# yknishidate/single-file-vulkan-pathtracing

Hardware: AMD Instinct MI355X
Metric: Mrays/s, Cornell Box 1920x1080 @ 8 bounces (ms/frame in ms_per_step) (higher is better)
Workload: dtype f32; 1 GPU; C2: CornellBox-Original.obj 1920x1080, 32 spp/frame x 774 frames, 8 bounces, fused pipeline (library default); pipeline=fused

## Files before the change

single-file-vulkan-pathtracing_amd/csrc/film_work.hip:

```cpp
#include "wavefront_host.h"

#include <algorithm>
#include <cmath>
#include <string>
#include <vector>

namespace {
using ptw::SPILL_POOL_ENTRIES;

constexpr size_t SLOT_BYTES_QUEUES = 2 * (8 + 16 + 16 + 8) + 16 + 4, SLOT_BYTES_META = 4 + 4;
constexpr size_t SLOT_BYTES = SLOT_BYTES_QUEUES + SLOT_BYTES_META;

struct WorkNeed { size_t slots, color, terms, terms_over, total; };
WorkNeed work_need(uint64_t n_slots, uint32_t groups, uint32_t term_cap, uint32_t term_pcap, bool queues = true, uint32_t tail = 0)
{
    WorkNeed n{};
    const size_t heads = (size_t)std::max<uint64_t>(n_slots, 1);
    n.slots = tail ? heads * tail : heads;
    n.color = groups == 1 ? heads : 0;
    const bool logs = groups > 1 || tail;
    n.terms = logs ? n.slots * (size_t)term_pcap : 0;
    n.terms_over = logs ? n.slots * (size_t)(term_cap - term_pcap) : 0;
    n.total = n.slots * (queues ? SLOT_BYTES : SLOT_BYTES_META) + sizeof(float4) * (n.color + n.terms + n.terms_over) +
              (logs ? sizeof(float4) * (size_t)SPILL_POOL_ENTRIES : 0);
// ... 50 lines not shown
            for (uint32_t tx = 0; tx < tiles_x; tx++)
                if ((tx + ty) % world == rank) tiles.push_back(tx | (ty << 16));
        if (order == 1u) {
            auto ring = [&](uint32_t t) {
                const float cx = 0.5f * (float)tiles_x, cy = 0.5f * (float)tiles_y;
                const float dx = std::fabs(((float)(t & 0xFFFFu) + 0.5f) - cx) / cx, dy = std::fabs(((float)(t >> 16) + 0.5f) - cy) / cy;
                return std::max(dx, dy);
            };
            std::stable_sort(tiles.begin(), tiles.end(), [&](uint32_t a, uint32_t b) { return ring(a) < ring(b); });
        }
        w.tile_order = order;
        w.rank = rank; w.world = world;
        w.n_tiles = (uint32_t)tiles.size();
        w.tile_rect[0] = w.tile_rect[1] = 0; w.tile_rect[2] = w.tile_rect[3] = -1;
        if (order == 1u) w.h_tiles = tiles; else w.h_tiles.clear();
        PT_HIP(ctx, hipMalloc((void **)&w.d_tiles, sizeof(uint32_t) * std::max<size_t>(tiles.size(), 1)));
        if (!tiles.empty())
            PT_HIP(ctx, hipMemcpy(w.d_tiles, tiles.data(), sizeof(uint32_t) * tiles.size(), hipMemcpyHostToDevice));
    }
    const uint64_t n_slots64 = (uint64_t)lanes * groups * w.n_tiles * 64ull;
    if (n_slots64 >= (1ull << 31)) {
        ctx->err = "too many path slots (frames_in_flight x sample_groups x pixels >= 2^31)";
        return PT_ERR_INVALID_ARG;
    }
    if (!w.d_count) PT_HIP(ctx, hipMalloc((void **)&w.d_count, sizeof(uint32_t) * PTW_COUNT_WORDS));
    if (tail && (n_slots64 * tail >= (1ull << 31) || queues || groups != 1)) {
        ctx->err = "head + tail slots: too many tail slots, or not the fused pipeline's one-group shape";
        return PT_ERR_INVALID_ARG;
    }
    const WorkNeed need = work_need(n_slots64, groups, term_cap, term_pcap, queues, tail);
    const size_t ns = need.slots;
    const size_t limit = ctx->mem_budget;
    pt_status rc = PT_OK;
// ... 148 lines not shown
    std::vector<uint32_t> out;
    out.reserve(w.h_tiles.size());
    if (none) {
        out = w.h_tiles;
    } else {
        auto touches = [&](uint32_t t) {
            const int32_t x = (int32_t)(t & 0xFFFFu) * 8, y = (int32_t)(t >> 16) * 8;
            return x <= rect[2] && x + 7 >= rect[0] && y <= rect[3] && y + 7 >= rect[1];
        };
        for (uint32_t t : w.h_tiles) if (touches(t)) out.push_back(t);
        for (uint32_t t : w.h_tiles) if (!touches(t)) out.push_back(t);
    }
    PT_HIP(ctx, hipStreamSynchronize(st));
    PT_HIP(ctx, hipMemcpy(w.d_tiles, out.data(), sizeof(uint32_t) * out.size(), hipMemcpyHostToDevice));
    std::copy(rect, rect + 4, w.tile_rect);
    return PT_OK;
}

pt_status ptw_shape_and_work(pt_film *f, const pt_params *p_in, RenderShape &sh, int launch_class, bool queues)
{
    pt_status rc = PT_OK;
    pt_params p_local = *p_in;
    if (p_local.pipeline == PT_PIPELINE_WAVEFRONT_NEE) p_local.sample_groups = 1;
    const pt_params *p = &p_local;
    for (int attempt = 0; attempt < 12; attempt++) {
        sh = ptw_choose_shape(f, p, launch_class, attempt);
        rc = ptw_ensure_work(f, p->rank, p->world, sh.lanes, sh.groups, sh.term_cap, sh.term_pcap, queues);
        if (rc != PT_ERR_OOM) return rc;
        const bool can_shrink = (p->frames_in_flight == 0 && sh.lanes > 1) || (p->sample_groups == 0 && sh.groups > 1);
        if (!can_shrink) return rc;
// ... 71 lines not shown
```

single-file-vulkan-pathtracing_amd/csrc/fused.hip:

```cpp
#include "wavefront_host.h"

#include <algorithm>

#define PT_EXTEND_TEMPLATES_ONLY
#include "extend_kernel.h"
#include "extend_inst16.h"

#ifdef PT_FUSED_TIMELINE
__device__ unsigned long long *g_fused_timeline = nullptr;
extern "C" int pt_debug_fused_timeline(void *device_u64x4_per_wave)
{
    return (int)hipMemcpyToSymbol(HIP_SYMBOL(g_fused_timeline), &device_u64x4_per_wave, sizeof(void *));
}
#endif

#ifdef PT_FUSED_HIST
__device__ uint32_t *g_fused_hist = nullptr;
extern "C" int pt_debug_fused_hist(void *device_u32_2x8192x16)
{
    return (int)hipMemcpyToSymbol(HIP_SYMBOL(g_fused_hist), &device_u32_2x8192x16, sizeof(void *));
}
#endif

#include "fused_cull.h"
// ... 83 lines not shown
{
    pt_ctx *ctx = s->ctx;
    if (s->n_inst && nee) {
        ctx->err = "PT_PIPELINE_FUSED with PT_FLAG_NEE is for single-level scenes (instanced scenes: PT_PIPELINE_WAVEFRONT_NEE)";
        return PT_ERR_UNSUPPORTED;
    }
    if (s->n_inst) return plan_fused_inst(s, pl, tmin, fp);
    const size_t tables = sizeof(float4) * 5 * (size_t)s->n_tris;
    if (pl.variant != PT_EXTEND_LDS || pl.spill || !(tmin > 0.f) || tables > 16 * 1024) {
        ctx->err = "PT_PIPELINE_FUSED is for single-level scenes whose BVH4, triangles and shading tables fit LDS (the compact "
                   "kernels' class: <= 2047 triangles in <= 24 KB, stack bound <= 16, tmin > 0)";
        return PT_ERR_UNSUPPORTED;
    }
    fp.lds_stack = pl.lds_stack + 1;
    fp.smem = (size_t)fp.lds_stack * FTB * sizeof(uint32_t) + lds_scene_bytes(s->n_wide, s->n_tris) + tables +
              sizeof(uint32_t) * FS_FIELDS * FTB + sizeof(uint32_t) * (FTB / 64) * PT_FUSED_WTILES;
    fp.pairs = pl.pairs;
    fp.block = FTB;
    int per_cu = 0;
    pt_status rcp;
    if (nee) {
        fp.nee = true;
        fp.smem += sizeof(uint32_t) * FS_NEE_FIELDS * FTB;
        rcp = fused_blocks_per_cu(ctx, 2, fp.smem, pl.pairs, per_cu,
                                  [&](int *n) { return ptw_prepare_kernel(ctx, reinterpret_cast<const void *>(pick_fused_nee(pl.pairs)), FTB, fp.smem, n); });
    } else {
        rcp = fused_blocks_per_cu(ctx, 0, fp.smem, pl.pairs, per_cu, [&](int *n) {
            pt_status rc = PT_OK;
            for (int mode = 2; mode >= 0 && rc == PT_OK; mode--) {
                rc = ptw_prepare_kernel(ctx, reinterpret_cast<const void *>(pick_fused(mode, pl.pairs, true)), FTB, fp.smem + FUSED_COUNT_LDS);
                if (rc == PT_OK) rc = ptw_prepare_kernel(ctx, reinterpret_cast<const void *>(pick_fused(mode, pl.pairs, false)), FTB, fp.smem, mode == 0 ? n : nullptr);
// ... 38 lines not shown
```

single-file-vulkan-pathtracing_amd/csrc/fused_kernel.h:

```cpp
#pragma once

#ifndef PT_FUSED_WAVES
#define PT_FUSED_WAVES 6
#endif

#ifndef PT_FUSED_TB
#define PT_FUSED_TB 512
#endif
constexpr int FTB = PT_FUSED_TB;

#ifndef PT_FUSED_BATCH
#define PT_FUSED_BATCH 256
#endif
#ifndef PT_FUSED_BATCH1
#define PT_FUSED_BATCH1 64
#endif
#define PT_FUSED_WTILES (PT_FUSED_BATCH / 64)
#define PT_FUSED_PARTS 8
#define PT_FUSED_PART_STRIDE 32

enum : int { FS_SLOT = 0, FS_CTR, FS_SEED, FS_WR, FS_WG, FS_WB, FS_PXY, FS_A, FS_B, FS_C, FS_MB, FS_FIELDS };
enum : int { FS_NEE_POS = 0, FS_NEE_R, FS_NEE_G, FS_NEE_B, FS_NEE_FIELDS };
#ifndef PT_FUSED_WAVES_NEE
#define PT_FUSED_WAVES_NEE 4
#endif

#ifndef PT_FUSED_NODE_EXIT
#define PT_FUSED_NODE_EXIT 3
#endif
#ifndef PT_FUSED_NODE_EXIT_B
#define PT_FUSED_NODE_EXIT_B 1
#endif
enum FusedBlock : int {
    FB_ITER = 0,
    FB_SHADE,
    FB_HIT,
    FB_MISS,
// ... 55 lines not shown
    float4 *s_shade = s_tri + 9 * (size_t)n_tris;
    float4 *s_frame = s_shade + 3 * (size_t)n_tris;
    lds_u32 *my_state = (lds_u32 *)reinterpret_cast<uint32_t *>(s_frame + 2 * (size_t)n_tris) + threadIdx.x;
    lds_stage_nodes<FTB, true>(s_wide, g_wide, n_wide);
    lds_stage_tris<FTB, true>(s_tri, g_tri4, n_tris, s_shade, g_shade4);
    for (uint32_t i = threadIdx.x; i < 2 * n_tris; i += FTB) s_frame[i] = g_frame4[i];
    __syncthreads();
    const float4 *wide = s_wide, *tri4 = s_tri;
    const float4 *verts = s_tri + 6 * (size_t)n_tris;

    lds_u32 *my_stack32 = (lds_u32 *)reinterpret_cast<uint32_t *>(smem) + FTB + threadIdx.x;
    const int lane = threadIdx.x & 63;

    FusedDev dev;
    dev.kernel_begin();
    lds_u32 *s_fb = (lds_u32 *)reinterpret_cast<uint32_t *>(s_frame + 2 * (size_t)n_tris) + FS_FIELDS * FTB + (FTB / 64) * PT_FUSED_WTILES + (threadIdx.x >> 6) * (2 * FB_N);
    if constexpr (COUNT) {
        if (lane < 2 * FB_N) s_fb[lane] = 0u;
    }
#define PT_FB(B)                                                                                        \
    if constexpr (COUNT) {                                                                              \
        const unsigned long long m_fb = __ballot(1);                                                    \
        if (lane == __ffsll((long long)m_fb) - 1) { s_fb[2 * (B)] += 1u; s_fb[2 * (B) + 1] += (uint32_t)__popcll(m_fb); } \
    }
    bool out_of_slots = false;
    uint32_t n_rays_wave = 0;
    uint32_t n_cull_wave = 0;
    uint32_t w_next = 0, w_end = 0, w_base = 0;
    uint32_t w_part = blockIdx.x % (uint32_t)PT_FUSED_PARTS, w_tried = 0;
    bool w_tails = false;
    const uint32_t n_tail_slots = HYB ? rc.lanes_active * rc.tail * rc.slots_per_lane : 0u;
    const uint32_t part_len = ((n_slots + PT_FUSED_PARTS - 1) / PT_FUSED_PARTS + 63u) & ~63u;
    lds_u32 *s_wtile = (lds_u32 *)reinterpret_cast<uint32_t *>(s_frame + 2 * (size_t)n_tris) + FS_FIELDS * FTB + (threadIdx.x >> 6) * PT_FUSED_WTILES;
    lds_u32 *my_nee = (lds_u32 *)reinterpret_cast<uint32_t *>(s_frame + 2 * (size_t)n_tris) + FS_FIELDS * FTB + (FTB / 64) * PT_FUSED_WTILES + threadIdx.x;
    ptm::f3 inv{}, invf{}, on{}, of{}, orgp{};
    ptm::RayPre pre{};
    uint32_t ax = 0, ay = 0, az = 0, tri_base = 0;
    float best_t = tmax, best_V = 0.f, best_W = 0.f, best_det = 1.f;
    uint32_t best_pos = PT_MISS;
    uint32_t cur = DONE;
    int sp = -1;

    constexpr uint32_t PENDING = 0xFFFFFFFFu;
    auto pop_pending = [&](uint32_t r) -> uint32_t {
        while (__ballot(r == PENDING)) {
            if (r == PENDING) {
                PT_FB(FB_POP)
                sp--;
                const uint32_t e = my_stack32[sp * FTB];
// ... 150 lines not shown
                        w_part = (w_part + 1u) % (uint32_t)PT_FUSED_PARTS;
                        if (++w_tried >= (uint32_t)PT_FUSED_PARTS) {
                            if (HYB && !w_tails && n_tail_slots) {
                                w_tails = true;
                                w_tried = 0;
                                w_part = blockIdx.x % (uint32_t)PT_FUSED_PARTS;
                                continue;
                            }
                            out_of_slots = true;
                            w_end = w_next;
                            break;
                        }
                    }
                    if (out_of_slots) dev.out_of_slots();
                    if (!out_of_slots && (uint32_t)lane < (w_end - w_base + 63u) / 64u) {
                        if (GROUPED || (HYB && w_tails)) {
                            const uint32_t c = slot_base + w_base + 64u * (uint32_t)lane;
                            s_wtile[lane] = tiles[(c - rc.div_spl.div(c) * rc.slots_per_lane) >> 6];
                        } else {
                            s_wtile[lane] = tiles[div_frames.div(((w_base >> 6) + (uint32_t)lane) * (uint32_t)PT_FUSED_PARTS + w_part)];
                        }
                    }
                    __builtin_amdgcn_wave_barrier();
                }
                const uint32_t take = min((uint32_t)__popcll(m_want), w_end - w_next);
                const uint32_t rank = (uint32_t)__popcll(m_want & ((1ull << lane) - 1ull));
                uint32_t cull_n = 0u;
                if (in_blk && sp < 0 && rank < take) {
                    PT_FB(FB_TAKE)
                    const uint32_t mine = w_next + rank;
                    uint32_t f, g, local;
                    if (HYB && w_tails) {
                        const uint32_t lane_slot = rc.div_spl.div(mine);
                        f = rc.div_tail.div(lane_slot); g = lane_slot - f * rc.tail;
                        local = mine - lane_slot * rc.slots_per_lane;
                        slot = rc.n_head + mine;
                    } else if (GROUPED) {
                        slot = slot_base + mine;
                        const uint32_t lane_slot = rc.div_spl.div(slot);
                        f = rc.div_groups.div(lane_slot); g = lane_slot - f * rc.groups;
                        local = slot - lane_slot * rc.slots_per_lane;
                    } else {
                        const uint32_t q = (mine >> 6) * (uint32_t)PT_FUSED_PARTS + w_part;
                        const uint32_t t = div_frames.div(q);
                        f = q - t * rc.lanes_active; g = 0u;
                        local = t * 64u + (mine & 63u);
                        slot = slot_base + f * rc.slots_per_lane + local;
                    }
                    const uint32_t tw = s_wtile[(mine - w_base) >> 6];
                    const uint32_t px = (tw & 0xFFFFu) * 8u + (local & 7u), py = (tw >> 16) * 8u + ((local >> 3) & 7u);
                    const uint32_t sample0 = (HYB && w_tails) ? rc.head_samples + g : g * rc.group_size;
                    const bool in_image = px < rc.width && py < rc.height && f < rc.lanes_active && sample0 < rc.spp;
                    if (in_image && ptc::pixel_culled(rc, px, py)) {
                        PT_FB(FB_CULLED)
                        if (GROUPED) cull_n = ptc::finish_group(rc, rad, slot, g);
                        else if (!(HYB && w_tails)) cull_n = ptc::finish_plain(rc, rad, slot);
                    } else if (in_image) {
                        pxy = px | (py << 16);
                        ctr = sample0;
                        my_state[FS_A * FTB] = 0u;
                        if (!GROUPED) { my_state[FS_B * FTB] = 0u; my_state[FS_C * FTB] = 0u; }
                        my_state[FS_MB * FTB] = (uint32_t)((int32_t)rc.spp * (rc.frame_base + (int32_t)f)) + 1u;
                        sp = 0;
                        need_primary = true;
                        dev.slot_begin();
                    } else if (GROUPED) {
                        rad.nterm[slot] = 0u;
                    } else if (HYB && w_tails) {
                        rad.nterm[slot - rc.n_head] = 0u;
                    }
                }
                w_next += take;
                if (rc.cull_on) {
                    const uint32_t n_c = ptc::rays_finished<GROUPED>(rc, cull_n);
                    n_rays_wave += n_c;
                    n_cull_wave += n_c;
                }
// ... 54 lines not shown
                    if (shadow) {
                        my_nee[FS_NEE_R * FTB] = __float_as_uint(nc.x); my_nee[FS_NEE_G * FTB] = __float_as_uint(nc.y); my_nee[FS_NEE_B * FTB] = __float_as_uint(nc.z);
                    }
                }
                pre = ptm::ray_setup<true>(org, dir);
                inv = { ptm::safe_inv(dir.x), ptm::safe_inv(dir.y), ptm::safe_inv(dir.z) };
                slab_setup(org, inv, invf, on, of);
                ax = inv.x < 0.f ? 48u : 0u;
                ay = inv.y < 0.f ? 48u : 0u;
                az = inv.z < 0.f ? 48u : 0u;
                tri_base = (uint32_t)pre.kz * 3u * n_tris;
                orgp = { ptm::sel3(pre.kz, org.y, org.z, org.x), ptm::sel3(pre.kz, org.z, org.x, org.y), ptm::sel3(pre.kz, org.x, org.y, org.z) };
                best_t = (NEE && shadow) ? nc.w : tmax;
                best_V = 0.f; best_W = 0.f; best_det = 1.f;
                best_pos = PT_MISS;
                cur = 0u;
                sp = 0;
            }
            const uint32_t n_started = (uint32_t)__popcll(__ballot(got_ray));
            n_rays_wave += n_started;
            dev.rays_started(n_started, HYB && w_tails, lane);
        }
        const bool tracing = cur != DONE;
        const unsigned long long m_tracing = __ballot(tracing);
        if (m_tracing == 0ull && __ballot(sp >= 0) == 0ull && out_of_slots) break;

        const int n_have = __popcll(m_tracing);
        if (tracing) { PT_FB(FB_TRACE) }
        {
            bool dn = cur < LEAF_BIT;
            if (__ballot(dn) != 0ull) {
// ... 102 lines not shown
```

single-file-vulkan-pathtracing_amd/csrc/pt_internal.h:

```cpp
#pragma once
#include <hip/hip_runtime.h>
#include <stdint.h>

#include <string>
#include <vector>

#include "../../include/pt_api.h"

constexpr int PT_N_STATS = 24;
constexpr int PT_N_BLOCKS = 32;
constexpr int PT_N_STATS_ALL = PT_N_STATS + 2 * PT_N_BLOCKS;
constexpr int PT_MAX_PIPES = 4;
namespace {
constexpr int TB = 256;
constexpr uint32_t SENTINEL = 0xFFFFFFFFu;
}

struct pt_ctx {
    int device = 0;
    hipStream_t stream = nullptr;
    bool own_stream = false;
    int num_cus = 256;
    std::string err;
    unsigned long long *d_stats = nullptr;
// ... 65 lines not shown
    std::vector<uint32_t> h_light_prim;
    std::vector<float> h_xforms;
    float4 *d_lights_inst = nullptr;
    uint32_t n_lights_inst = 0;
    float light_area_inst = 0.f;
    uint32_t n_inst = 0, n_tlas_wide = 0, tlas_height = 0;
    double tlas_area_lbvh = 0.0, tlas_area_ploc = 0.0;
    float4 *d_inst6 = nullptr;
    float4 *d_inst_frame = nullptr;
    float4 *d_tlas_wide = nullptr;
    uint32_t *d_tlas_prim_of = nullptr;
    uint4 *d_tlas16 = nullptr;
    uint32_t n_tlas16 = 0, tlas16_levels = 0;
    float tlas_norm_c[3]{}, tlas_norm_s[3]{1.f, 1.f, 1.f}, tlas_norm_rs[3]{1.f, 1.f, 1.f};
    float tlas_bmin[3]{}, tlas_bmax[3]{};
};

struct pt_film {
    pt_ctx *ctx = nullptr;
    uint32_t w = 0, h = 0;
    float *d_rgb = nullptr;
    bool own_rgb = true;
    uint8_t *d_bgra = nullptr;
    struct Work {
        uint32_t rank = 0, world = 0, lanes = 0;
        uint32_t tile_order = 0;
        uint32_t groups = 0, term_cap = 0;
        uint32_t tail = 0;
        uint32_t n_tiles = 0;
        uint32_t n_slots = 0;
        uint32_t *d_tiles = nullptr;
        std::vector<uint32_t> h_tiles;
        int32_t tile_rect[4] = { 0, 0, -1, -1 };
        float4 *d_color = nullptr;
        float4 *d_terms = nullptr;
        float4 *d_terms_over = nullptr;
        uint32_t *d_nterm = nullptr;
        uint32_t *d_spill_head = nullptr;
        float4 *d_spill = nullptr;
        uint2 *d_qid[2] = { nullptr, nullptr };
        float4 *d_qstate[2] = { nullptr, nullptr };
        float4 *d_qrayA[2] = { nullptr, nullptr };
        float2 *d_qrayB[2] = { nullptr, nullptr };
        float4 *d_hit = nullptr;
        uint32_t *d_hit_inst = nullptr;
        uint32_t *d_count = nullptr;
// ... 71 lines not shown
```

single-file-vulkan-pathtracing_amd/csrc/render.hip:

```cpp
#include "wavefront_host.h"

#include <cstring>
#include <algorithm>
#include <string>
#include <vector>

namespace {
using namespace ptw;

pt_status check_params(pt_scene *s, pt_film *f, const pt_params *p)
{
    pt_ctx *ctx = s->ctx;
    if (p->width != f->w || p->height != f->h) { ctx->err = "params width/height differ from the film's"; return PT_ERR_INVALID_ARG; }
    if (p->world == 0 || p->rank >= p->world) { ctx->err = "rank/world invalid"; return PT_ERR_INVALID_ARG; }
    if (p->spp_per_frame == 0 || p->spp_per_frame > 0xFFFFu || p->max_depth == 0 || p->max_depth > 0xFFFFu) {
        ctx->err = "spp_per_frame and max_depth must be in 1..65535";
        return PT_ERR_INVALID_ARG;
    }
    if (p->frame < 0 || p->frame_count == 0) { ctx->err = "frame must be >= 0 and frame_count >= 1"; return PT_ERR_INVALID_ARG; }
    if (p->pipeline > PT_PIPELINE_AUTO) { ctx->err = "unknown pipeline"; return PT_ERR_UNSUPPORTED; }
    if (p->pipeline == PT_PIPELINE_FUSED && (p->flags & PT_FLAG_ASYNC)) {
        ctx->err = "the fused pipeline has no asynchronous form";
        return PT_ERR_UNSUPPORTED;
    }
// ... 88 lines not shown
    }
    const float size[2] = { (float)p->width, (float)p->height };
    int32_t r[4];
    for (int k = 0; k < 2; k++) {
        const float a = (lo[k] + 1.0f) * 0.5f * size[k] - 1.0f, b = (hi[k] + 1.0f) * 0.5f * size[k] + 1.0f;
        if (!(a == a) || !(b == b) || b < 0.f || a > size[k]) return;
        r[k] = (int32_t)std::max(a, 0.f);
        r[k + 2] = (int32_t)std::min(b, size[k] - 1.0f);
    }
    std::copy(r, r + 4, rect);
}

void apply_cull(const pt_ctx *ctx, const pt_params *p, const int32_t rect[4], RenderConst &rc)
{
    rc.cull_on = 0u;
    if (rect[2] < rect[0] || rect[3] < rect[1] || ctx->tune.cull == 0 || ((p->flags & PT_FLAG_COUNT_VISITS) && ctx->tune.cull != 1)) return;
    if (!std::isfinite(p->env[0]) || !std::isfinite(p->env[1]) || !std::isfinite(p->env[2])) return;
    rc.cull_on = 1u;
    std::copy(rect, rect + 4, rc.cull);
    for (int k = 0; k < 3; k++) {
        volatile float c = 0.0f;
        for (uint32_t i = 0; i < p->spp_per_frame; i++) c = c + 1.0f * p->env[k];
        rc.cull_sum[k] = c;
    }
}

pt_status job_setup(Job &j)
{
    pt_scene *s = j.s; pt_film *f = j.f; const pt_params *p = j.p; pt_ctx *ctx = j.ctx;
    pt_film::Work &w = f->work;
    const uint32_t lanes = j.sh.lanes, groups = j.sh.groups;
// ... 451 lines not shown
    if (ctx->tune.term_spill >= 0) spill_cap = std::min<uint32_t>(spill_cap, (uint32_t)ctx->tune.term_spill);
    static_assert(sizeof(Radiance) <= sizeof(pt_ctx::h_rad), "pt_ctx::h_rad holds a Radiance");
    Radiance rad{};
    auto set_rad = [&]() -> pt_status {
        rad = { w.d_color, w.d_terms, w.d_terms_over, w.d_nterm, w.d_spill, w.d_spill_head, d_spill_count, spill_cap, d_overflow, static_cast<const Radiance *>(ctx->d_rad) };
        if (std::memcmp(ctx->h_rad, &rad, sizeof(rad)) != 0) {
            std::memcpy(ctx->h_rad, &rad, sizeof(rad));
            PT_HIP(ctx, hipMemcpyAsync(ctx->d_rad, ctx->h_rad, sizeof(rad), hipMemcpyHostToDevice, st));
        }
        return PT_OK;
    };
    rc_ = set_rad();
    if (rc_ != PT_OK) return rc_;
    RenderConst rc = ptw_render_const(p, w, sh);
    apply_cull(ctx, p, rect, rc);
    const bool profile = !nested && (p->flags & PT_FLAG_PROFILE) != 0;
    ctx->stats.extend_variant = pl.variant;
    ctx->stats.pipelines = 1;
    if (!nested) PT_HIP(ctx, hipEventRecord(ctx->ev_a, st));
    std::vector<hipEvent_t> evs;
    size_t ev_used = 0;
    for (uint32_t done = 0; w.n_slots > 0 && done < p->frame_count; done += sh.lanes) {
        rc.frame_base = p->frame + (int32_t)done;
        rc.lanes_active = std::min(sh.lanes, p->frame_count - done);
        unsigned long long *const d_rays_before = ctx->d_stats + 18;
        if (sh.bounded) {
            PT_HIP(ctx, hipMemcpyAsync(d_rays_before, ctx->d_stats, sizeof(unsigned long long), hipMemcpyDeviceToDevice, st));
            PT_HIP(ctx, hipMemcpyAsync(ctx->d_stats + 20, ctx->d_stats + 19, sizeof(unsigned long long), hipMemcpyDeviceToDevice, st));
            PT_HIP(ctx, hipMemsetAsync(d_spill_count, 0, sizeof(unsigned long long), st));
        }
// ... 112 lines not shown
    if (rc_ != PT_OK) return rc_;
    rc_ = check_params(s, f, p_in);
    if (rc_ != PT_OK) return rc_;
    ExtendPlan pl;
    rc_ = ptw_plan_extend(s, p_in->extend, pl);
    if (rc_ != PT_OK) return rc_;
    pt_params p_res = *p_in;
    p_res.pipeline = resolve_pipeline(s, p_in, pl);
    const pt_params *p = &p_res;
    s->ctx->stats.pipeline = p->pipeline;
    if (p->pipeline == PT_PIPELINE_FUSED) return render_fused(s, f, p, pl, false, false);
    return render_wavefront(s, f, p, pl, false);
}

void ptw_subject_rect(const pt_scene *s, const pt_params *p, int32_t rect[4]) { subject_rect(s, p, rect); }

pt_status ptw_trace(pt_scene *s, const float *rays6, uint32_t n, float tmin, float tmax, uint32_t extend, pt_hit *hits)
{
    pt_ctx *ctx = s->ctx;
    hipStream_t st = ctx->stream;
    if (n == 0) return PT_OK;
    ExtendPlan pl;
    pt_status rc_ = ptw_plan_extend(s, extend, pl);
    if (rc_ != PT_OK) return rc_;
    std::vector<float4> a(n);
    std::vector<float2> b(n);
    for (uint32_t i = 0; i < n; i++) {
        const float *r = rays6 + 6 * (size_t)i;
        a[i] = make_float4(r[0], r[1], r[2], r[3]);
        b[i] = make_float2(r[4], r[5]);
// ... 37 lines not shown
```

single-file-vulkan-pathtracing_amd/csrc/scene_build.hip:

```cpp
#include "bvh_build.h"

#include <hip/hip_fp16.h>

#include <algorithm>
#include <cmath>
#include <cstdlib>
#include <cstring>
#include <string>
#include <vector>

namespace {

__global__ __launch_bounds__(TB) void k_gather(const float *__restrict__ vertices, const uint32_t *__restrict__ indices,
                                               uint32_t n_tris, float4 *__restrict__ tri_orig,
                                               float4 *__restrict__ tlo, float4 *__restrict__ thi)
{
    const uint32_t t = blockIdx.x * TB + threadIdx.x;
    float mn[3] = { INFINITY, INFINITY, INFINITY }, mx[3] = { -INFINITY, -INFINITY, -INFINITY };
    if (t < n_tris) {
        float v[3][3];
        for (int c = 0; c < 3; c++) {
            const uint32_t vi = indices[3 * (size_t)t + c];
            for (int k = 0; k < 3; k++) v[c][k] = vertices[3 * (size_t)vi + k];
        }
// ... 71 lines not shown
        for (int k = 0; k < 4; k++) {
            hl[k] = __half_as_ushort(__float2half_rd((l[k] - c[ax]) * rs[ax] - 3.814697265625e-06f));
            hh[k] = __half_as_ushort(__float2half_ru((h[k] - c[ax]) * rs[ax] + 3.814697265625e-06f));
        }
        d[2 * ax + 0] = hl[0] | (hl[1] << 16); d[2 * ax + 1] = hl[2] | (hl[3] << 16);
        d[6 + 2 * ax + 0] = hh[0] | (hh[1] << 16); d[6 + 2 * ax + 1] = hh[2] | (hh[3] << 16);
    }
    const float4 cw = nd[6];
    uint4 *o = out + 4 * (size_t)i;
    o[0] = make_uint4(d[0], d[1], d[2], d[3]);
    o[1] = make_uint4(d[4], d[5], d[6], d[7]);
    o[2] = make_uint4(d[8], d[9], d[10], d[11]);
    o[3] = make_uint4(__float_as_uint(cw.x), __float_as_uint(cw.y), __float_as_uint(cw.z), __float_as_uint(cw.w));
}

static pt_status make_wide16(pt_scene *s)
{
    pt_ctx *ctx = s->ctx;
    hipStream_t st = ctx->stream;
    ptb_norm_box(s->bmin, s->bmax, s->norm_c, s->norm_s, s->norm_rs);
    (void)hipFree(s->d_wide16);
    s->d_wide16 = nullptr;
    PT_HIP(ctx, hipMalloc((void **)&s->d_wide16, 64 * (size_t)s->n_wide));
    k_wide_half<<<(s->n_wide + TB - 1) / TB, TB, 0, st>>>(s->d_wide, s->n_wide, s->norm_c[0], s->norm_c[1], s->norm_c[2], s->norm_rs[0],
                                                         s->norm_rs[1], s->norm_rs[2], reinterpret_cast<uint4 *>(s->d_wide16));
    PT_HIP(ctx, hipStreamSynchronize(st));
    PT_HIP(ctx, hipGetLastError());
    return PT_OK;
}

__global__ __launch_bounds__(TB) void k_tri_boxes(const float4 *__restrict__ tri_orig, uint32_t n, float4 *__restrict__ tlo,
                                                  float4 *__restrict__ thi)
{
    const uint32_t t = blockIdx.x * TB + threadIdx.x;
    if (t >= n) return;
    const float4 a = tri_orig[3 * (size_t)t + 0], b = tri_orig[3 * (size_t)t + 1], c = tri_orig[3 * (size_t)t + 2];
    tlo[t] = make_float4(fminf(fminf(a.x, b.x), c.x), fminf(fminf(a.y, b.y), c.y), fminf(fminf(a.z, b.z), c.z), 0.f);
    thi[t] = make_float4(fmaxf(fmaxf(a.x, b.x), c.x), fmaxf(fmaxf(a.y, b.y), c.y), fmaxf(fmaxf(a.z, b.z), c.z), 0.f);
}

static void free_tree_products(pt_scene *s)
{
    (void)hipFree(s->d_nodes); (void)hipFree(s->d_keys); (void)hipFree(s->d_prim_of); (void)hipFree(s->d_prim_of_sah);
// ... 499 lines not shown
    if (rc == PT_OK && s->d_wide_sah)
        rc = ptb_refit_wide(ctx, 0, s->d_wide_sah, s->n_wide_sah, d_tlo, d_thi, s->d_prim_of_sah, n, pad, s->norm_c, s->norm_rs);
    if (rc == PT_OK && s->d_wide16t)
        rc = ptb_refit_wide(ctx, 1, s->d_wide16t, s->n_wide16t, d_tlo, d_thi, kept, n, pad, s->norm_c, s->norm_rs);
    if (rc == PT_OK && s->d_wide8)
        rc = ptb_refit_wide(ctx, 2, s->d_wide8, s->n_wide8, d_tlo, d_thi, s->d_prim_of8, n, pad, s->norm_c, s->norm_rs);
    if (rc != PT_OK) return rc;
    const uint32_t *order = s->bvh4_builder != 0u ? s->d_prim_of_sah : s->d_prim_of;
    if (s->d_wide8)
        k_pack<<<gt, TB, 0, st>>>(s->d_tri_orig, s->d_faces, s->d_prim_of8, n, s->d_tri4_8, s->d_shade4, s->d_shade64_8, s->d_ke4_8);
    k_pack<<<gt, TB, 0, st>>>(s->d_tri_orig, s->d_faces, order, n, s->d_tri4, s->d_shade4, s->d_shade64, s->d_ke4, s->d_frame4);
    k_wide_half<<<(s->n_wide + TB - 1) / TB, TB, 0, st>>>(s->d_wide, s->n_wide, s->norm_c[0], s->norm_c[1], s->norm_c[2], s->norm_rs[0],
                                                         s->norm_rs[1], s->norm_rs[2], reinterpret_cast<uint4 *>(s->d_wide16));
    PT_HIP(ctx, hipGetLastError());
    PT_HIP(ctx, hipStreamSynchronize(st));
    return PT_OK;
}

static void keep_host_boxes(pt_scene *s, const std::vector<float4> &lo, const std::vector<float4> &hi)
{
    const uint32_t n = s->n_tris;
    s->h_tlo.resize(3 * (size_t)n);
    s->h_thi.resize(3 * (size_t)n);
    for (uint32_t i = 0; i < n; i++) {
        s->h_tlo[3 * i + 0] = lo[i].x; s->h_tlo[3 * i + 1] = lo[i].y; s->h_tlo[3 * i + 2] = lo[i].z;
        s->h_thi[3 * i + 0] = hi[i].x; s->h_thi[3 * i + 1] = hi[i].y; s->h_thi[3 * i + 2] = hi[i].z;
    }
}

static pt_status update_tree_products(pt_scene *s, const float4 *d_tlo, const float4 *d_thi, bool refit)
{
// ... 83 lines not shown
```

single-file-vulkan-pathtracing_amd/csrc/wavefront_host.h:

```cpp
#pragma once
#include "wavefront_types.h"

#include <hip/hip_ext.h>

#include <algorithm>

inline pt_status ptw_reserve_spill(pt_ctx *ctx, size_t bytes)
{
    if (bytes <= ctx->spill_bytes) return PT_OK;
    (void)hipFree(ctx->d_spill);
    ctx->d_spill = nullptr;
    ctx->spill_bytes = 0;
    PT_HIP(ctx, hipMalloc((void **)&ctx->d_spill, bytes));
    ctx->spill_bytes = bytes;
    return PT_OK;
}
inline pt_status ptw_prepare_kernel(pt_ctx *ctx, const void *fn, int block, size_t smem, int *per_cu = nullptr)
{
    if (smem > 48 * 1024) PT_HIP(ctx, hipFuncSetAttribute(fn, hipFuncAttributeMaxDynamicSharedMemorySize, (int)smem));
    if (!per_cu) return PT_OK;
    PT_HIP(ctx, hipOccupancyMaxActiveBlocksPerMultiprocessor(per_cu, fn, block, smem));
    *per_cu = std::max(1, std::min(*per_cu, 8));
    return PT_OK;
}
// ... 70 lines not shown
pt_status ptw_plan_fused(pt_scene *s, const ExtendPlan &pl, float tmin, FusedPlan &fp, bool nee = false);
void ptw_launch_fused(const FusedPlan &fp, bool grouped, const ptw::RenderConst &rc, const uint32_t *tiles, const ptw::Radiance &rad,
                      const pt_scene *s, uint32_t n_slots, uint32_t *next_slot, unsigned long long *stats, float tmin, float tmax,
                      hipStream_t st, hipEvent_t ev0, hipEvent_t ev1);

struct RenderShape {
    uint32_t lanes = 1, groups = 1, group_size = 1, term_cap = 0, term_pcap = 0;
    bool bounded = false;
    uint32_t tail = 0;
};
RenderShape ptw_choose_shape(const pt_film *f, const pt_params *p, int launch_class, int shrink = 0);
pt_status ptw_ensure_work(pt_film *f, uint32_t rank, uint32_t world, uint32_t lanes, uint32_t groups, uint32_t term_cap, uint32_t term_pcap,
                          bool queues = true, uint32_t tail = 0);
pt_status ptw_shape_and_work(pt_film *f, const pt_params *p, RenderShape &sh, int launch_class, bool queues = true);
pt_status ptw_tiles_subject_first(pt_film *f, const int32_t rect[4], hipStream_t st);
uint64_t ptw_workspace_bytes(const pt_film *f);
ptw::RenderConst ptw_render_const(const pt_params *p, const pt_film::Work &w, const RenderShape &sh);
uint64_t ptw_valid_local_pixels(const pt_film *f, const pt_params *p);
void ptw_subject_rect(const pt_scene *s, const pt_params *p, int32_t rect[4]);

const void *ptw_extend_hbm_fn(bool count, bool rec64);
void ptw_launch_extend_hbm(bool count, bool rec64, int grid, size_t smem, hipStream_t st, hipEvent_t ev0, hipEvent_t ev1,
                           const float4 *wide, const uint2 *wide16, const float *norm_c, const float *norm_s,
                           const float *norm_rs, const float4 *tri4, const float4 *rec64_tab, uint32_t n_wide, uint32_t n_tris,
                           const float4 *rayA, const float2 *rayB, float4 *hit, const uint32_t *count_in, uint32_t *count_zero,
                           unsigned long long *stats, uint2 *spill, uint32_t spill_stride, int refill, float tmin,
                           float tmax, int lds_stack, int raw_hit, const uint32_t *perm, const float *ray_tmax);
const void *ptw_extend8_fn(bool count, bool spills, bool waves7);
void ptw_launch_extend8(bool count, bool spills, bool waves7, int grid, size_t smem, hipStream_t st, hipEvent_t ev0, hipEvent_t ev1, const uint4 *nodes8,
                        const float *norm_c, const float *norm_s, const float *norm_rs, const float4 *tri4, const float4 *rec64, const float4 *rayA,
// ... 7 lines not shown
```

Before: 58600 Mrays/s.

## Start primary-ray traversal at a precomputed per-tile BVH leaf

After each BVH build, the host reads back the wide BVH and records which leaf holds each triangle. Per frame, it projects all triangles onto the screen and tags each 8x8 tile that only one leaf covers. The tags are stored in a second plane of the tile buffer and staged through LDS. Primary rays in a tagged tile start traversal at that leaf instead of the root, skipping the top-level walk. This adds host readback and classification work on scene or camera changes, plus extra LDS per block. It relies on a simplified camera projection that must match the device camera model.

```diff
diff --git a/single-file-vulkan-pathtracing_amd/csrc/film_work.hip b/single-file-vulkan-pathtracing_amd/csrc/film_work.hip
--- a/single-file-vulkan-pathtracing_amd/csrc/film_work.hip
+++ b/single-file-vulkan-pathtracing_amd/csrc/film_work.hip
@@ -1,7 +1,9 @@
 #include "wavefront_host.h"
+#include "first_leaf.h"
 
 #include <algorithm>
 #include <cmath>
+#include <cstring>
 #include <string>
 #include <vector>
 
@@ -88,9 +90,12 @@
         w.n_tiles = (uint32_t)tiles.size();
         w.tile_rect[0] = w.tile_rect[1] = 0; w.tile_rect[2] = w.tile_rect[3] = -1;
         if (order == 1u) w.h_tiles = tiles; else w.h_tiles.clear();
-        PT_HIP(ctx, hipMalloc((void **)&w.d_tiles, sizeof(uint32_t) * std::max<size_t>(tiles.size(), 1)));
+        PT_HIP(ctx, hipMalloc((void **)&w.d_tiles, sizeof(uint32_t) * 2 * std::max<size_t>(tiles.size(), 1)));
+        PT_HIP(ctx, hipMemset(w.d_tiles, 0, sizeof(uint32_t) * 2 * std::max<size_t>(tiles.size(), 1)));
         if (!tiles.empty())
             PT_HIP(ctx, hipMemcpy(w.d_tiles, tiles.data(), sizeof(uint32_t) * tiles.size(), hipMemcpyHostToDevice));
+        w.h_order = tiles;
+        w.leaf_gen = 0; w.leaf_stale = false; w.leaf_tiles = 0;
     }
     const uint64_t n_slots64 = (uint64_t)lanes * groups * w.n_tiles * 64ull;
     if (n_slots64 >= (1ull << 31)) {
@@ -269,6 +274,37 @@
     PT_HIP(ctx, hipStreamSynchronize(st));
     PT_HIP(ctx, hipMemcpy(w.d_tiles, out.data(), sizeof(uint32_t) * out.size(), hipMemcpyHostToDevice));
     std::copy(rect, rect + 4, w.tile_rect);
+    w.h_order = out;
+    w.leaf_stale = w.leaf_gen != 0;
+    return PT_OK;
+}
+
+pt_status ptw_tiles_first_leaf(pt_film *f, const pt_scene *s, const pt_params *p, bool on, hipStream_t st)
+{
+    pt_film::Work &w = f->work;
+    pt_ctx *ctx = f->ctx;
+    if (!w.d_tiles || !w.n_tiles) return PT_OK;
+    uint32_t *plane = w.d_tiles + w.n_tiles;
+    on = on && s->h_leaf_of.size() == s->n_tris && w.h_order.size() == w.n_tiles;
+    if (!on) {
+        if (w.leaf_gen != 0 || w.leaf_stale) {
+            PT_HIP(ctx, hipStreamSynchronize(st));
+            PT_HIP(ctx, hipMemset(plane, 0, sizeof(uint32_t) * w.n_tiles));
+        }
+        w.leaf_gen = 0; w.leaf_stale = false; w.leaf_tiles = 0;
+        return PT_OK;
+    }
+    const float cam[6] = { p->cam_origin[0], p->cam_origin[1], p->cam_origin[2], p->cam_target[0], p->cam_target[1], p->cam_target[2] };
+    if (!w.leaf_stale && w.leaf_gen == s->tree_gen && std::memcmp(cam, w.leaf_cam, sizeof(cam)) == 0 && w.leaf_size[0] == p->width && w.leaf_size[1] == p->height)
+        return PT_OK;
+    std::vector<uint32_t> codes(w.n_tiles);
+    w.leaf_tiles = ptf::classify_tiles(s->h_leaf_tri9.data(), s->h_leaf_of.data(), s->n_tris, p->cam_origin, p->cam_target, p->width, p->height,
+                                       w.h_order.data(), w.n_tiles, codes.data());
+    PT_HIP(ctx, hipStreamSynchronize(st));
+    PT_HIP(ctx, hipMemcpy(plane, codes.data(), sizeof(uint32_t) * w.n_tiles, hipMemcpyHostToDevice));
+    w.leaf_gen = s->tree_gen; w.leaf_stale = false;
+    std::memcpy(w.leaf_cam, cam, sizeof(cam));
+    w.leaf_size[0] = p->width; w.leaf_size[1] = p->height;
     return PT_OK;
 }
 
diff --git a/single-file-vulkan-pathtracing_amd/csrc/first_leaf.h b/single-file-vulkan-pathtracing_amd/csrc/first_leaf.h
--- /dev/null
+++ b/single-file-vulkan-pathtracing_amd/csrc/first_leaf.h
@@ -0,0 +1,77 @@
+#pragma once
+#include <stdint.h>
+
+#include <algorithm>
+#include <cmath>
+#include <vector>
+
+namespace ptf {
+
+constexpr uint32_t NONE = 0u;
+
+inline uint32_t classify_tiles(const float *tri9, const uint32_t *leaf_of, uint32_t n_tris, const float cam_origin[3], const float cam_target[3],
+                               uint32_t width, uint32_t height, const uint32_t *tiles, uint32_t n_tiles, uint32_t *codes)
+{
+    std::fill(codes, codes + n_tiles, NONE);
+    const double o[3] = { cam_origin[0], cam_origin[1], cam_origin[2] }, t[3] = { cam_target[0], cam_target[1], cam_target[2] };
+    const double den = t[2] - o[2], size[2] = { (double)width, (double)height };
+    if (!(std::fabs(den) > 0.0) || !n_tris || !width || !height) return 0u;
+    std::vector<double> img(6 * (size_t)n_tris);
+    for (uint32_t i = 0; i < 3 * n_tris; i++) {
+        const float *P = tri9 + 3 * (size_t)i;
+        const double a = ((double)P[2] - o[2]) / den;
+        if (!(a > 1.0e-4)) return 0u;
+        for (int k = 0; k < 2; k++) {
+            const double d = o[k] + ((double)P[k] - o[k]) / a - t[k];
+            const double s = (d + 1.0) * 0.5 * size[k];
+            if (!std::isfinite(s)) return 0u;
+            img[2 * (size_t)i + k] = s;
+        }
+    }
+    const int32_t tiles_x = (int32_t)((width + 7) / 8), tiles_y = (int32_t)((height + 7) / 8);
+    constexpr uint32_t MANY = 0xFFFFFFFFu;
+    std::vector<uint32_t> grid((size_t)tiles_x * tiles_y, NONE);
+    for (uint32_t i = 0; i < n_tris; i++) {
+        const double *v = &img[6 * (size_t)i];
+        double big = 0.0;
+        for (int k = 0; k < 6; k++) big = std::max(big, std::fabs(v[k]));
+        const double slack = 1.0 + big * (1.0 / 1048576.0);
+        const double ylo = std::min({ v[1], v[3], v[5] }), yhi = std::max({ v[1], v[3], v[5] });
+        const int32_t ty0 = (int32_t)std::clamp(std::floor((ylo - slack - 8.0) / 8.0), 0.0, (double)tiles_y),
+                      ty1 = (int32_t)std::clamp(std::ceil((yhi + slack) / 8.0), -1.0, (double)tiles_y - 1.0);
+        for (int32_t ty = ty0; ty <= ty1; ty++) {
+            const double ya = 8.0 * ty - slack, yb = 8.0 * ty + 8.0 + slack;
+            if (yhi < ya || ylo > yb) continue;
+            double xlo = 1.0e300, xhi = -1.0e300;
+            for (int e = 0; e < 3; e++) {
+                const double ax = v[2 * e], ay = v[2 * e + 1], bx = v[2 * ((e + 1) % 3)], by = v[2 * ((e + 1) % 3) + 1];
+                if (ay >= ya && ay <= yb) { xlo = std::min(xlo, ax); xhi = std::max(xhi, ax); }
+                for (const double yl : { ya, yb }) {
+                    if ((ay < yl) != (by < yl)) {
+                        const double x = ax + (bx - ax) * ((yl - ay) / (by - ay));
+                        xlo = std::min(xlo, std::clamp(x, std::min(ax, bx), std::max(ax, bx)));
+                        xhi = std::max(xhi, std::clamp(x, std::min(ax, bx), std::max(ax, bx)));
+                    }
+                }
+            }
+            if (xlo > xhi) continue;
+            const int32_t tx0 = (int32_t)std::clamp(std::floor((xlo - slack - 8.0) / 8.0), 0.0, (double)tiles_x),
+                          tx1 = (int32_t)std::clamp(std::ceil((xhi + slack) / 8.0), -1.0, (double)tiles_x - 1.0);
+            for (int32_t tx = tx0; tx <= tx1; tx++) {
+                if (xhi < 8.0 * tx - slack || xlo > 8.0 * tx + 8.0 + slack) continue;
+                uint32_t &g = grid[(size_t)ty * tiles_x + tx];
+                g = (g == NONE || g == leaf_of[i]) ? leaf_of[i] : MANY;
+            }
+        }
+    }
+    uint32_t n = 0;
+    for (uint32_t k = 0; k < n_tiles; k++) {
+        const uint32_t tx = tiles[k] & 0xFFFFu, ty = tiles[k] >> 16;
+        if ((int32_t)tx >= tiles_x || (int32_t)ty >= tiles_y) continue;
+        const uint32_t g = grid[(size_t)ty * tiles_x + tx];
+        if (g != NONE && g != MANY) { codes[k] = g; n++; }
+    }
+    return n;
+}
+
+}
diff --git a/single-file-vulkan-pathtracing_amd/csrc/fused.hip b/single-file-vulkan-pathtracing_amd/csrc/fused.hip
--- a/single-file-vulkan-pathtracing_amd/csrc/fused.hip
+++ b/single-file-vulkan-pathtracing_amd/csrc/fused.hip
@@ -121,7 +121,7 @@
     }
     fp.lds_stack = pl.lds_stack + 1;
     fp.smem = (size_t)fp.lds_stack * FTB * sizeof(uint32_t) + lds_scene_bytes(s->n_wide, s->n_tris) + tables +
-              sizeof(uint32_t) * FS_FIELDS * FTB + sizeof(uint32_t) * (FTB / 64) * PT_FUSED_WTILES;
+              sizeof(uint32_t) * FS_TAIL_AT;
     fp.pairs = pl.pairs;
     fp.block = FTB;
     int per_cu = 0;
diff --git a/single-file-vulkan-pathtracing_amd/csrc/fused_kernel.h b/single-file-vulkan-pathtracing_amd/csrc/fused_kernel.h
--- a/single-file-vulkan-pathtracing_amd/csrc/fused_kernel.h
+++ b/single-file-vulkan-pathtracing_amd/csrc/fused_kernel.h
@@ -16,11 +16,14 @@
 #define PT_FUSED_BATCH1 64
 #endif
 #define PT_FUSED_WTILES (PT_FUSED_BATCH / 64)
+#define PT_FUSED_WTILE_WORDS (2 * PT_FUSED_WTILES)
 #define PT_FUSED_PARTS 8
 #define PT_FUSED_PART_STRIDE 32
 
 enum : int { FS_SLOT = 0, FS_CTR, FS_SEED, FS_WR, FS_WG, FS_WB, FS_PXY, FS_A, FS_B, FS_C, FS_MB, FS_FIELDS };
 enum : int { FS_NEE_POS = 0, FS_NEE_R, FS_NEE_G, FS_NEE_B, FS_NEE_FIELDS };
+constexpr int FS_LEAF_AT = FS_FIELDS * PT_FUSED_TB + (PT_FUSED_TB / 64) * PT_FUSED_WTILE_WORDS;
+constexpr int FS_TAIL_AT = FS_LEAF_AT + PT_FUSED_TB;
 #ifndef PT_FUSED_WAVES_NEE
 #define PT_FUSED_WAVES_NEE 4
 #endif
@@ -106,7 +109,7 @@
 
     FusedDev dev;
     dev.kernel_begin();
-    lds_u32 *s_fb = (lds_u32 *)reinterpret_cast<uint32_t *>(s_frame + 2 * (size_t)n_tris) + FS_FIELDS * FTB + (FTB / 64) * PT_FUSED_WTILES + (threadIdx.x >> 6) * (2 * FB_N);
+    lds_u32 *s_fb = (lds_u32 *)reinterpret_cast<uint32_t *>(s_frame + 2 * (size_t)n_tris) + FS_TAIL_AT + (threadIdx.x >> 6) * (2 * FB_N);
     if constexpr (COUNT) {
         if (lane < 2 * FB_N) s_fb[lane] = 0u;
     }
@@ -123,8 +126,8 @@
     bool w_tails = false;
     const uint32_t n_tail_slots = HYB ? rc.lanes_active * rc.tail * rc.slots_per_lane : 0u;
     const uint32_t part_len = ((n_slots + PT_FUSED_PARTS - 1) / PT_FUSED_PARTS + 63u) & ~63u;
-    lds_u32 *s_wtile = (lds_u32 *)reinterpret_cast<uint32_t *>(s_frame + 2 * (size_t)n_tris) + FS_FIELDS * FTB + (threadIdx.x >> 6) * PT_FUSED_WTILES;
-    lds_u32 *my_nee = (lds_u32 *)reinterpret_cast<uint32_t *>(s_frame + 2 * (size_t)n_tris) + FS_FIELDS * FTB + (FTB / 64) * PT_FUSED_WTILES + threadIdx.x;
+    lds_u32 *s_wtile = (lds_u32 *)reinterpret_cast<uint32_t *>(s_frame + 2 * (size_t)n_tris) + FS_FIELDS * FTB + (threadIdx.x >> 6) * PT_FUSED_WTILE_WORDS;
+    lds_u32 *my_nee = (lds_u32 *)reinterpret_cast<uint32_t *>(s_frame + 2 * (size_t)n_tris) + FS_TAIL_AT + threadIdx.x;
     ptm::f3 inv{}, invf{}, on{}, of{}, orgp{};
     ptm::RayPre pre{};
     uint32_t ax = 0, ay = 0, az = 0, tri_base = 0;
@@ -305,12 +308,15 @@
                     }
                     if (out_of_slots) dev.out_of_slots();
                     if (!out_of_slots && (uint32_t)lane < (w_end - w_base + 63u) / 64u) {
+                        uint32_t t;
                         if (GROUPED || (HYB && w_tails)) {
                             const uint32_t c = slot_base + w_base + 64u * (uint32_t)lane;
-                            s_wtile[lane] = tiles[(c - rc.div_spl.div(c) * rc.slots_per_lane) >> 6];
+                            t = (c - rc.div_spl.div(c) * rc.slots_per_lane) >> 6;
                         } else {
-                            s_wtile[lane] = tiles[div_frames.div(((w_base >> 6) + (uint32_t)lane) * (uint32_t)PT_FUSED_PARTS + w_part)];
-                        }
+                            t = div_frames.div(((w_base >> 6) + (uint32_t)lane) * (uint32_t)PT_FUSED_PARTS + w_part);
+                        }
+                        s_wtile[lane] = tiles[t];
+                        s_wtile[PT_FUSED_WTILES + lane] = tiles[(rc.slots_per_lane >> 6) + t];
                     }
                     __builtin_amdgcn_wave_barrier();
                 }
@@ -338,7 +344,7 @@
                         local = t * 64u + (mine & 63u);
                         slot = slot_base + f * rc.slots_per_lane + local;
                     }
-                    const uint32_t tw = s_wtile[(mine - w_base) >> 6];
+                    const uint32_t tw = s_wtile[(mine - w_base) >> 6], tleaf = s_wtile[PT_FUSED_WTILES + ((mine - w_base) >> 6)];
                     const uint32_t px = (tw & 0xFFFFu) * 8u + (local & 7u), py = (tw >> 16) * 8u + ((local >> 3) & 7u);
                     const uint32_t sample0 = (HYB && w_tails) ? rc.head_samples + g : g * rc.group_size;
                     const bool in_image = px < rc.width && py < rc.height && f < rc.lanes_active && sample0 < rc.spp;
@@ -352,6 +358,7 @@
                         my_state[FS_A * FTB] = 0u;
                         if (!GROUPED) { my_state[FS_B * FTB] = 0u; my_state[FS_C * FTB] = 0u; }
                         my_state[FS_MB * FTB] = (uint32_t)((int32_t)rc.spp * (rc.frame_base + (int32_t)f)) + 1u;
+                        my_state[FS_LEAF_AT] = tleaf;
                         sp = 0;
                         need_primary = true;
                         dev.slot_begin();
@@ -436,7 +443,7 @@
                 best_t = (NEE && shadow) ? nc.w : tmax;
                 best_V = 0.f; best_W = 0.f; best_det = 1.f;
                 best_pos = PT_MISS;
-                cur = 0u;
+                cur = need_primary ? (uint32_t)my_state[FS_LEAF_AT] : 0u;
                 sp = 0;
             }
             const uint32_t n_started = (uint32_t)__popcll(__ballot(got_ray));
diff --git a/single-file-vulkan-pathtracing_amd/csrc/pt_internal.h b/single-file-vulkan-pathtracing_amd/csrc/pt_internal.h
--- a/single-file-vulkan-pathtracing_amd/csrc/pt_internal.h
+++ b/single-file-vulkan-pathtracing_amd/csrc/pt_internal.h
@@ -103,6 +103,9 @@
     uint32_t n_tlas16 = 0, tlas16_levels = 0;
     float tlas_norm_c[3]{}, tlas_norm_s[3]{1.f, 1.f, 1.f}, tlas_norm_rs[3]{1.f, 1.f, 1.f};
     float tlas_bmin[3]{}, tlas_bmax[3]{};
+    std::vector<uint32_t> h_leaf_of;
+    std::vector<float> h_leaf_tri9;
+    uint64_t tree_gen = 0;
 };
 
 struct pt_film {
@@ -119,6 +122,12 @@
         uint32_t n_tiles = 0;
         uint32_t n_slots = 0;
         uint32_t *d_tiles = nullptr;
+        std::vector<uint32_t> h_order;
+        uint64_t leaf_gen = 0;
+        float leaf_cam[6] = {};
+        uint32_t leaf_size[2] = { 0, 0 };
+        bool leaf_stale = false;
+        uint32_t leaf_tiles = 0;
         std::vector<uint32_t> h_tiles;
         int32_t tile_rect[4] = { 0, 0, -1, -1 };
         float4 *d_color = nullptr;
diff --git a/single-file-vulkan-pathtracing_amd/csrc/render.hip b/single-file-vulkan-pathtracing_amd/csrc/render.hip
--- a/single-file-vulkan-pathtracing_amd/csrc/render.hip
+++ b/single-file-vulkan-pathtracing_amd/csrc/render.hip
@@ -1,4 +1,5 @@
 #include "wavefront_host.h"
+#include "first_leaf.h"
 
 #include <cstring>
 #include <algorithm>
@@ -126,7 +127,7 @@
 void apply_cull(const pt_ctx *ctx, const pt_params *p, const int32_t rect[4], RenderConst &rc)
 {
     rc.cull_on = 0u;
-    if (rect[2] < rect[0] || rect[3] < rect[1] || ctx->tune.cull == 0 || ((p->flags & PT_FLAG_COUNT_VISITS) && ctx->tune.cull != 1)) return;
+    if (rect[2] < rect[0] || rect[3] < rect[1] || ctx->tune.cull == 0 || ((p->flags & PT_FLAG_COUNT_VISITS) && ctx->tune.cull < 1)) return;
     if (!std::isfinite(p->env[0]) || !std::isfinite(p->env[1]) || !std::isfinite(p->env[2])) return;
     rc.cull_on = 1u;
     std::copy(rect, rect + 4, rc.cull);
@@ -608,6 +609,8 @@
     if (rc_ != PT_OK) return rc_;
     RenderConst rc = ptw_render_const(p, w, sh);
     apply_cull(ctx, p, rect, rc);
+    rc_ = ptw_tiles_first_leaf(f, s, p, !fp.inst && rc.cull_on && ctx->tune.cull != 2, st);
+    if (rc_ != PT_OK) return rc_;
     const bool profile = !nested && (p->flags & PT_FLAG_PROFILE) != 0;
     ctx->stats.extend_variant = pl.variant;
     ctx->stats.pipelines = 1;
@@ -750,6 +753,12 @@
 }
 
 void ptw_subject_rect(const pt_scene *s, const pt_params *p, int32_t rect[4]) { subject_rect(s, p, rect); }
+
+extern "C" uint32_t pt_debug_first_leaf_tiles(const float *tri9, const uint32_t *leaf_of, uint32_t n_tris, const float *cam_origin, const float *cam_target,
+                                              uint32_t width, uint32_t height, const uint32_t *tiles, uint32_t n_tiles, uint32_t *codes)
+{
+    return ptf::classify_tiles(tri9, leaf_of, n_tris, cam_origin, cam_target, width, height, tiles, n_tiles, codes);
+}
 
 pt_status ptw_trace(pt_scene *s, const float *rays6, uint32_t n, float tmin, float tmax, uint32_t extend, pt_hit *hits)
 {
diff --git a/single-file-vulkan-pathtracing_amd/csrc/scene_build.hip b/single-file-vulkan-pathtracing_amd/csrc/scene_build.hip
--- a/single-file-vulkan-pathtracing_amd/csrc/scene_build.hip
+++ b/single-file-vulkan-pathtracing_amd/csrc/scene_build.hip
@@ -1,8 +1,10 @@
 #include "bvh_build.h"
+#include "lds_scene.h"
 
 #include <hip/hip_fp16.h>
 
 #include <algorithm>
+#include <atomic>
 #include <cmath>
 #include <cstdlib>
 #include <cstring>
@@ -109,6 +111,41 @@
     o[3] = make_uint4(__float_as_uint(cw.x), __float_as_uint(cw.y), __float_as_uint(cw.z), __float_as_uint(cw.w));
 }
 
+static pt_status ptb_read_leaf_map(pt_scene *s)
+{
+    static std::atomic<uint64_t> builds{ 0 };
+    pt_ctx *ctx = s->ctx;
+    s->tree_gen = ++builds;
+    s->h_leaf_of.clear();
+    s->h_leaf_tri9.clear();
+    const uint32_t n = s->n_tris;
+    if (!n || n > 2047u || !s->n_wide || s->n_wide > 0x1FFFu || !s->d_wide || !s->d_tri4) return PT_OK;
+    std::vector<float4> wide(8 * (size_t)s->n_wide), tri(3 * (size_t)n);
+    PT_HIP(ctx, hipMemcpy(wide.data(), s->d_wide, sizeof(float4) * wide.size(), hipMemcpyDeviceToHost));
+    PT_HIP(ctx, hipMemcpy(tri.data(), s->d_tri4, sizeof(float4) * tri.size(), hipMemcpyDeviceToHost));
+    std::vector<uint32_t> leaf_of(n, 0u);
+    bool whole = true;
+    for (uint32_t i = 0; i < s->n_wide; i++) {
+        const float4 cw = wide[8 * (size_t)i + 6];
+        for (const float cf : { cw.x, cw.y, cw.z, cw.w }) {
+            uint32_t w;
+            std::memcpy(&w, &cf, sizeof(w));
+            if (w == SENTINEL || !(w & PT_LEAF)) continue;
+            const uint32_t first = w & 0x7FFu, more = (w >> 28) & 3u;
+            for (uint32_t k = first; k <= first + more; k++) {
+                if (k >= n || leaf_of[k]) { whole = false; break; }
+                leaf_of[k] = C14_LEAF | (more << 11) | first;
+            }
+        }
+    }
+    for (uint32_t k = 0; k < n; k++) whole = whole && leaf_of[k] != 0u;
+    if (!whole) return PT_OK;
+    s->h_leaf_tri9.resize(9 * (size_t)n);
+    for (uint32_t k = 0; k < 3 * n; k++) { s->h_leaf_tri9[3 * k + 0] = tri[k].x; s->h_leaf_tri9[3 * k + 1] = tri[k].y; s->h_leaf_tri9[3 * k + 2] = tri[k].z; }
+    s->h_leaf_of = leaf_of;
+    return PT_OK;
+}
+
 static pt_status make_wide16(pt_scene *s)
 {
     pt_ctx *ctx = s->ctx;
@@ -121,7 +158,7 @@
                                                          s->norm_rs[1], s->norm_rs[2], reinterpret_cast<uint4 *>(s->d_wide16));
     PT_HIP(ctx, hipStreamSynchronize(st));
     PT_HIP(ctx, hipGetLastError());
-    return PT_OK;
+    return ptb_read_leaf_map(s);
 }
 
 __global__ __launch_bounds__(TB) void k_tri_boxes(const float4 *__restrict__ tri_orig, uint32_t n, float4 *__restrict__ tlo,
@@ -651,7 +688,7 @@
                                                          s->norm_rs[1], s->norm_rs[2], reinterpret_cast<uint4 *>(s->d_wide16));
     PT_HIP(ctx, hipGetLastError());
     PT_HIP(ctx, hipStreamSynchronize(st));
-    return PT_OK;
+    return ptb_read_leaf_map(s);
 }
 
 static void keep_host_boxes(pt_scene *s, const std::vector<float4> &lo, const std::vector<float4> &hi)
diff --git a/single-file-vulkan-pathtracing_amd/csrc/wavefront_host.h b/single-file-vulkan-pathtracing_amd/csrc/wavefront_host.h
--- a/single-file-vulkan-pathtracing_amd/csrc/wavefront_host.h
+++ b/single-file-vulkan-pathtracing_amd/csrc/wavefront_host.h
@@ -108,6 +108,7 @@
                           bool queues = true, uint32_t tail = 0);
 pt_status ptw_shape_and_work(pt_film *f, const pt_params *p, RenderShape &sh, int launch_class, bool queues = true);
 pt_status ptw_tiles_subject_first(pt_film *f, const int32_t rect[4], hipStream_t st);
+pt_status ptw_tiles_first_leaf(pt_film *f, const pt_scene *s, const pt_params *p, bool on, hipStream_t st);
 uint64_t ptw_workspace_bytes(const pt_film *f);
 ptw::RenderConst ptw_render_const(const pt_params *p, const pt_film::Work &w, const RenderShape &sh);
 uint64_t ptw_valid_local_pixels(const pt_film *f, const pt_params *p);
```

Result: slower. 49730 Mrays/s (-15.1%).
